# vislearn/esac

Hardware: NVIDIA H100
Metric: pose hypotheses scored/sec (640x480, 256 hyp x E experts) (higher is better)
Workload: dtype f32 (scoring) / f64 (P3P, refinement)

## Files before the change

esac_b200/csrc/esac_p3p_fast.cuh:

```cuda
#pragma once
#include "esac_geom.cuh"

namespace esacb200 {

struct Pack1 {
    float a;
    static constexpr int W = 1;
};
struct Mask1 {
    bool a;
};
struct Pack2 {
    float2 v;
    static constexpr int W = 2;
};
struct Mask2 {
    bool a, b;
};
template <typename P> struct MaskOf;
template <> struct MaskOf<Pack1> { typedef Mask1 type; };
template <> struct MaskOf<Pack2> { typedef Mask2 type; };

ESAC_HD Pack1 bc1(float x) { Pack1 r; r.a = x; return r; }
ESAC_HD Pack2 bc2(float x) { Pack2 r; r.v = make_float2(x, x); return r; }
template <typename P> ESAC_HD P bc(float x);
template <> ESAC_HD Pack1 bc<Pack1>(float x) { return bc1(x); }
template <> ESAC_HD Pack2 bc<Pack2>(float x) { return bc2(x); }

ESAC_HD Pack1 operator+(Pack1 x, Pack1 y) { return bc1(x.a + y.a); }
ESAC_HD Pack1 operator-(Pack1 x, Pack1 y) { return bc1(x.a - y.a); }
ESAC_HD Pack1 operator*(Pack1 x, Pack1 y) { return bc1(x.a * y.a); }
ESAC_HD Pack1 operator-(Pack1 x) { return bc1(-x.a); }
ESAC_HD Pack1 fma_(Pack1 x, Pack1 y, Pack1 z) { return bc1(fmaf(x.a, y.a, z.a)); }
#ifdef __CUDA_ARCH__
ESAC_HD Pack2 operator+(Pack2 x, Pack2 y) { Pack2 r; r.v = fadd2(x.v, y.v); return r; }
ESAC_HD Pack2 operator*(Pack2 x, Pack2 y) { Pack2 r; r.v = fmul2(x.v, y.v); return r; }
ESAC_HD Pack2 fma_(Pack2 x, Pack2 y, Pack2 z) { Pack2 r; r.v = ffma2(x.v, y.v, z.v); return r; }
ESAC_HD Pack2 operator-(Pack2 x, Pack2 y) { Pack2 r; r.v = ffma2(make_float2(-1.f, -1.f), y.v, x.v); return r; }
#else
ESAC_HD Pack2 operator+(Pack2 x, Pack2 y) { Pack2 r; r.v = make_float2(x.v.x + y.v.x, x.v.y + y.v.y); return r; }
ESAC_HD Pack2 operator*(Pack2 x, Pack2 y) { Pack2 r; r.v = make_float2(x.v.x * y.v.x, x.v.y * y.v.y); return r; }
ESAC_HD Pack2 fma_(Pack2 x, Pack2 y, Pack2 z) { Pack2 r; r.v = make_float2(fmaf(x.v.x, y.v.x, z.v.x), fmaf(x.v.y, y.v.y, z.v.y)); return r; }
ESAC_HD Pack2 operator-(Pack2 x, Pack2 y) { Pack2 r; r.v = make_float2(x.v.x - y.v.x, x.v.y - y.v.y); return r; }
#endif
ESAC_HD Pack2 operator-(Pack2 x) { Pack2 r; r.v = make_float2(-x.v.x, -x.v.y); return r; }

#define ESAC_PACK_UNARY(name, expr)                                                     \
    ESAC_HD Pack1 name(Pack1 p) { float x = p.a; return bc1(expr); }                    \
    ESAC_HD Pack2 name(Pack2 p) { Pack2 r; float x = p.v.x; r.v.x = (expr); x = p.v.y; r.v.y = (expr); return r; }
ESAC_PACK_UNARY(abs_, fabsf(x))
ESAC_PACK_UNARY(rcp_, Num<float>::div_(1.f, x))
ESAC_PACK_UNARY(sqrt_, Num<float>::sqrt_(x))
ESAC_PACK_UNARY(rsqrt_, rsqrtf(x))
ESAC_PACK_UNARY(cbrt_, cbrtf(x))
#undef ESAC_PACK_UNARY
ESAC_HD Pack1 max_(Pack1 x, Pack1 y) { return bc1(fmaxf(x.a, y.a)); }
ESAC_HD Pack1 min_(Pack1 x, Pack1 y) { return bc1(fminf(x.a, y.a)); }
ESAC_HD Pack2 max_(Pack2 x, Pack2 y) { Pack2 r; r.v = make_float2(fmaxf(x.v.x, y.v.x), fmaxf(x.v.y, y.v.y)); return r; }
ESAC_HD Pack2 min_(Pack2 x, Pack2 y) { Pack2 r; r.v = make_float2(fminf(x.v.x, y.v.x), fminf(x.v.y, y.v.y)); return r; }

#define ESAC_PACK_CMP(name, op)                                                       \
    ESAC_HD Mask1 name(Pack1 x, Pack1 y) { Mask1 m; m.a = x.a op y.a; return m; }     \
    ESAC_HD Mask2 name(Pack2 x, Pack2 y) { Mask2 m; m.a = x.v.x op y.v.x; m.b = x.v.y op y.v.y; return m; }
ESAC_PACK_CMP(lt_, <)
ESAC_PACK_CMP(le_, <=)
ESAC_PACK_CMP(gt_, >)
ESAC_PACK_CMP(ge_, >=)
#undef ESAC_PACK_CMP
ESAC_HD Mask1 operator&(Mask1 x, Mask1 y) { Mask1 m; m.a = x.a && y.a; return m; }
ESAC_HD Mask1 operator|(Mask1 x, Mask1 y) { Mask1 m; m.a = x.a || y.a; return m; }
ESAC_HD Mask1 operator!(Mask1 x) { Mask1 m; m.a = !x.a; return m; }
ESAC_HD Mask2 operator&(Mask2 x, Mask2 y) { Mask2 m; m.a = x.a && y.a; m.b = x.b && y.b; return m; }
ESAC_HD Mask2 operator|(Mask2 x, Mask2 y) { Mask2 m; m.a = x.a || y.a; m.b = x.b || y.b; return m; }
ESAC_HD Mask2 operator!(Mask2 x) { Mask2 m; m.a = !x.a; m.b = !x.b; return m; }
ESAC_HD Mask1 mask1(bool v) { Mask1 m; m.a = v; return m; }
ESAC_HD Mask2 mask2(bool v) { Mask2 m; m.a = v; m.b = v; return m; }
template <typename M> ESAC_HD M splat(bool v);
template <> ESAC_HD Mask1 splat<Mask1>(bool v) { return mask1(v); }
template <> ESAC_HD Mask2 splat<Mask2>(bool v) { return mask2(v); }
ESAC_HD bool all_(Mask1 m) { return m.a; }
ESAC_HD bool all_(Mask2 m) { return m.a && m.b; }
ESAC_HD Pack1 sel(Mask1 m, Pack1 x, Pack1 y) { return bc1(m.a ? x.a : y.a); }
ESAC_HD Pack2 sel(Mask2 m, Pack2 x, Pack2 y) { Pack2 r; r.v = make_float2(m.a ? x.v.x : y.v.x, m.b ? x.v.y : y.v.y); return r; }
ESAC_HD Mask1 nan_(Pack1 x) { return mask1(!(x.a == x.a)); }
ESAC_HD Mask2 nan_(Pack2 x) { Mask2 m; m.a = !(x.v.x == x.v.x); m.b = !(x.v.y == x.v.y); return m; }

template <typename P, typename M>
ESAC_HD void argmax3(P a0, P a1, P a2, M& is0, M& is1) {
    is0 = ge_(a0, a1) & ge_(a0, a2);
    is1 = !is0 & ge_(a1, a2);
}
template <typename P, typename M>
ESAC_HD P sel3(M is0, M is1, P v0, P v1, P v2) { return sel(is0, v0, sel(is1, v1, v2)); }

template <typename P, typename M>
ESAC_HD void fast_line_conic(P l0, P l1, P l2, P d00, P d01, P d02, P d11, P d12, P d22, P o[2][3], M& ok, M& unc) {
    using N = Num<float>;
    const P zero = bc<P>(0.f), one = bc<P>(1.f), two = bc<P>(2.f);
    const P a0 = abs_(l0), a1 = abs_(l1), a2 = abs_(l2);
    M k0, k1;
    argmax3(a0, a1, a2, k0, k1);
    const P li = sel3(k0, k1, l1, l2, l0), lj = sel3(k0, k1, l2, l0, l1), lk = sel3(k0, k1, l0, l1, l2);
    const M lk_ok = gt_(abs_(lk), zero);
    const P Dii = sel3(k0, k1, d11, d22, d00), Djj = sel3(k0, k1, d22, d00, d11), Dkk = sel3(k0, k1, d00, d11, d22);
    const P Dij = sel3(k0, k1, d12, d02, d01), Dik = sel3(k0, k1, d01, d12, d02), Djk = sel3(k0, k1, d02, d01, d12);
    const P ilk = rcp_(lk);
    const P r = li * ilk, s = lj * ilk;
    const P A = Dii - two * r * Dik + r * r * Dkk;
    const P B = Dij - s * Dik - r * Djk + r * s * Dkk;
    const P C = Djj - two * s * Djk + s * s * Dkk;
    P disc = B * B - A * C;
    const P mag = B * B + abs_(A * C);
    unc = unc | !lk_ok | (lk_ok & lt_(abs_(disc), bc<P>(N::kUncertain) * mag));
    const M real = !lt_(disc, -(bc<P>(N::kDiscTol) * mag));
    disc = max_(disc, zero);
    const P sq = sqrt_(disc);
    const P q = -(B + sel(ge_(B, zero), sq, -sq));
    const M useA = ge_(abs_(A), abs_(C));
    const P den = sel(useA, A, C), oth = sel(useA, C, A);
    const M den_ok = gt_(abs_(den), zero);
    unc = unc | (lk_ok & real & !den_ok);
    const P r0 = q * rcp_(den);
    const M q_nz = !(ge_(q, zero) & le_(q, zero));
    const P r1 = sel(q_nz, oth * rcp_(q), r0);
    ok = lk_ok & real & den_ok;
#pragma unroll
    for (int t = 0; t < 2; ++t) {
        const P rt = t == 0 ? r0 : r1;
        const P al = sel(useA, rt, one), be = sel(useA, one, rt);
        const P vi = al, vj = be, vk = -(r * al) - s * be;
        o[t][0] = sel3(k0, k1, vk, vj, vi);
        o[t][1] = sel3(k0, k1, vi, vk, vj);
        o[t][2] = sel3(k0, k1, vj, vi, vk);
    }
}

constexpr float kPrefilterMargin = 2.f;
constexpr float kPrefilterNeedle = 0.02f;

template <typename P>
ESAC_HD typename MaskOf<P>::type p3p_may_pass_pack(const P obj[4][3], const P img[4][2], float f, float ppx, float ppy, float tau,
                                                   float margin = kPrefilterMargin, float needle = kPrefilterNeedle) {
    typedef typename MaskOf<P>::type M;
    using N = Num<float>;
    const P zero = bc<P>(0.f), one = bc<P>(1.f), two = bc<P>(2.f);
    M decided = splat<M>(false), verdict = splat<M>(false);
#define ESAC_LATCH(cond, value)                         \
    {                                                   \
        const M c_ = (cond) & !decided;                 \
        verdict = (verdict & !c_) | (c_ & (value));     \
        decided = decided | c_;                         \
    }
    const M yes = splat<M>(true), no = splat<M>(false);
    P y[3][3], x1[3], x2[3], x3[3];
    const P ifx = bc<P>(N::div_(1.f, f)), vppx = bc<P>(ppx), vppy = bc<P>(ppy);
#pragma unroll
    for (int i = 0; i < 3; ++i) {
        const P bx = (img[i][0] - vppx) * ifx, by = (img[i][1] - vppy) * ifx;
        const P n = rsqrt_(fma_(bx, bx, fma_(by, by, one)));
        y[i][0] = bx * n; y[i][1] = by * n; y[i][2] = n;
    }
#pragma unroll
    for (int c = 0; c < 3; ++c) { x1[c] = obj[1][c] - obj[0][c]; x2[c] = obj[2][c] - obj[0][c]; x3[c] = obj[3][c] - obj[0][c]; }
    const P a12 = x1[0] * x1[0] + x1[1] * x1[1] + x1[2] * x1[2];
    const P a13 = x2[0] * x2[0] + x2[1] * x2[1] + x2[2] * x2[2];
    const P e0 = x1[0] - x2[0], e1 = x1[1] - x2[1], e2 = x1[2] - x2[2];
    const P a23 = e0 * e0 + e1 * e1 + e2 * e2;
    const P amax = max_(a12, max_(a13, a23)), amin = min_(a12, min_(a13, a23));
    ESAC_LATCH(nan_(amax), yes)
    ESAC_LATCH(!gt_(amax, zero), no)
    ESAC_LATCH(!lt_(amax, bc<P>(1e30f)), yes)
    const P c12 = y[0][0] * y[1][0] + y[0][1] * y[1][1] + y[0][2] * y[1][2];
    const P c13 = y[0][0] * y[2][0] + y[0][1] * y[2][1] + y[0][2] * y[2][2];
    const P c23 = y[1][0] * y[2][0] + y[1][1] * y[2][1] + y[1][2] * y[2][2];
    const P cm = max_(abs_(c12), max_(abs_(c13), abs_(c23)));
    ESAC_LATCH(lt_(amin, bc<P>(needle) * amax) | gt_(cm, bc<P>(0.9999f)), yes)
    const P iam = rcp_(amax);
    const P s12 = a12 * iam, s13 = a13 * iam, s23 = a23 * iam;
    const P p00 = s23, p01 = -(s23 * c12), p11 = s23 - s12, p12 = s12 * c23, p22 = -s12;
    const P q00 = s23, q02 = -(s23 * c13), q11 = -s13, q12 = s13 * c23, q22 = s23 - s13;
    const P P00 = p11 * p22 - p12 * p12, P01 = -(p01 * p22), P02 = p01 * p12;
    const P P11 = p00 * p22, P12 = -(p00 * p12), P22 = p00 * p11 - p01 * p01;
    const P Q00 = q11 * q22 - q12 * q12, Q01 = q02 * q12, Q02 = -(q02 * q11);
    const P Q11 = q00 * q22 - q02 * q02, Q12 = -(q00 * q12), Q22 = q00 * q11;
    const P k0 = p00 * P00 + p01 * P01;
    const P k3 = q00 * Q00 + q02 * Q02;
    const P k1 = P00 * q00 + P11 * q11 + P22 * q22 + two * (P02 * q02 + P12 * q12);
    const P k2 = Q00 * p00 + Q11 * p11 + Q22 * p22 + two * (Q01 * p01 + Q12 * p12);
    const P ksc = abs_(k3) + abs_(k2) + abs_(k1) + abs_(k0);
    ESAC_LATCH(!gt_(abs_(k3), bc<P>(1e-4f) * ksc), yes)
    const P ik3 = rcp_(k3);
    const P a = k2 * ik3, b = k1 * ik3, c = k0 * ik3;
    const P three = bc<P>(3.f);
    const P Qq = (a * a - three * b) * bc<P>(1.f / 9.f);
    const P Rr = (two * a * a * a - bc<P>(9.f) * a * b + bc<P>(27.f) * c) * bc<P>(1.f / 54.f);
    const P m3 = max_(sqrt_(abs_(Qq)), cbrt_(abs_(Rr)));
    P t = sel(gt_(Rr, zero), bc<P>(-2.002f), bc<P>(2.002f)) * m3;
#pragma unroll
    for (int it = 0; it < 10; ++it) {
        const P fv = (t * t - three * Qq) * t + two * Rr, dv = three * (t * t - Qq);
        t = t - sel(gt_(abs_(dv), zero), fv * rcp_(dv), zero);
    }
    P g = t - a * bc<P>(1.f / 3.f);
    {
        const P fv = ((g + a) * g + b) * g + c, dv = (three * g + two * a) * g + b;
        g = g - sel(gt_(abs_(dv), zero), fv * rcp_(dv), zero);
    }
    ESAC_LATCH(nan_(g), yes)
    const M small = le_(abs_(g), one);
    const P w1 = sel(small, one, rcp_(g)), w2 = sel(small, g, one);
    const P d00 = w1 * p00 + w2 * q00, d01 = w1 * p01, d02 = w2 * q02;
    const P d11 = w1 * p11 + w2 * q11, d12 = w1 * p12 + w2 * q12, d22 = w1 * p22 + w2 * q22;
    const P o00 = sel(small, q00, p00), o01 = sel(small, zero, p01), o02 = sel(small, q02, zero);
    const P o11 = sel(small, q11, p11), o12 = sel(small, q12, p12), o22 = sel(small, q22, p22);
    const P B00 = d11 * d22 - d12 * d12, B01 = d02 * d12 - d01 * d22, B02 = d01 * d12 - d02 * d11;
    const P B11 = d00 * d22 - d02 * d02, B12 = d01 * d02 - d00 * d12, B22 = d00 * d11 - d01 * d01;
    M ib0, ib1;
    argmax3(abs_(B00), abs_(B11), abs_(B22), ib0, ib1);
    const P bii = sel3(ib0, ib1, B00, B11, B22);
    const P nD = abs_(d00) + abs_(d11) + abs_(d22) + two * (abs_(d01) + abs_(d02) + abs_(d12));
    ESAC_LATCH(gt_(abs_(d00 * B00 + d01 * B01 + d02 * B02), bc<P>(1e-4f) * nD * nD * nD), yes)
    ESAC_LATCH(lt_(abs_(bii), bc<P>(N::kUncertain) * nD * nD), yes)
    ESAC_LATCH(!lt_(bii, zero), no)
    const P isq = rsqrt_(-bii);
    const P pv0 = sel3(ib0, ib1, B00, B01, B02) * isq, pv1 = sel3(ib0, ib1, B01, B11, B12) * isq, pv2 = sel3(ib0, ib1, B02, B12, B22) * isq;
    const P Cm[3][3] = {{d00, d01 - pv2, d02 + pv1}, {d01 + pv2, d11, d12 - pv0}, {d02 - pv1, d12 + pv0, d22}};
    P best = bc<P>(-1.f);
    P L0 = zero, L1 = zero, L2 = zero, M0 = zero, M1 = zero, M2 = zero;
#pragma unroll
    for (int r = 0; r < 3; ++r)
#pragma unroll
        for (int cc = 0; cc < 3; ++cc) {
            const P v = abs_(Cm[r][cc]);
            const M up = gt_(v, best);
            best = sel(up, v, best);
            L0 = sel(up, Cm[r][0], L0); L1 = sel(up, Cm[r][1], L1); L2 = sel(up, Cm[r][2], L2);
            M0 = sel(up, Cm[0][cc], M0); M1 = sel(up, Cm[1][cc], M1); M2 = sel(up, Cm[2][cc], M2);
        }
    ESAC_LATCH(!gt_(best, zero), yes)
    P dir[4][3];
    M unc = no, okL, okM;
    fast_line_conic(L0, L1, L2, o00, o01, o02, o11, o12, o22, &dir[0], okL, unc);
    fast_line_conic(M0, M1, M2, o00, o01, o02, o11, o12, o22, &dir[2], okM, unc);
    ESAC_LATCH(unc, yes)
    ESAC_LATCH(!okL & !okM, no)
    P nrm[3];
    nrm[0] = x1[1] * x2[2] - x1[2] * x2[1];
    nrm[1] = x1[2] * x2[0] - x1[0] * x2[2];
    nrm[2] = x1[0] * x2[1] - x1[1] * x2[0];
    const P g12 = x1[0] * x2[0] + x1[1] * x2[1] + x1[2] * x2[2];
    const P nn = nrm[0] * nrm[0] + nrm[1] * nrm[1] + nrm[2] * nrm[2];
    const P det = a12 * a13 - g12 * g12;
    ESAC_LATCH(!gt_(det, bc<P>(1e-6f) * a12 * a13) | !gt_(nn, zero), yes)
    const P v1 = x3[0] * x1[0] + x3[1] * x1[1] + x3[2] * x1[2], v2 = x3[0] * x2[0] + x3[1] * x2[1] + x3[2] * x2[2];
    const P idet = rcp_(det);
    const P al = (v1 * a13 - v2 * g12) * idet, be = (v2 * a12 - v1 * g12) * idet;
    const P ga = (x3[0] * nrm[0] + x3[1] * nrm[1] + x3[2] * nrm[2]) * rcp_(nn);
    const float lim = margin * tau;
    const P lim2 = bc<P>(lim * lim);
    const P sa = sqrt_(amax);
    const P vf = bc<P>(f);
    M pass = no;
#pragma unroll
    for (int s = 0; s < 4; ++s) {
        const M live = s < 2 ? okL : okM;
        P l0 = dir[s][0], l1 = dir[s][1], l2 = dir[s][2];
        const P q12 = l0 * l0 + l1 * l1 - two * c12 * l0 * l1;
        const P q13 = l0 * l0 + l2 * l2 - two * c13 * l0 * l2;
        const P q23 = l1 * l1 + l2 * l2 - two * c23 * l1 * l2;
        const M m12 = ge_(q12, q13) & ge_(q12, q23), m13 = !m12 & ge_(q13, q23);
        const P sc2 = sel3(m12, m13, s12, s13, s23) * rcp_(sel3(m12, m13, q12, q13, q23));
        const M scale_ok = gt_(sc2, zero) & lt_(sc2, bc<P>(1e30f));
        P sc = sqrt_(sc2);
        const P mx = max_(abs_(l0), max_(abs_(l1), abs_(l2)));
        const P ku = bc<P>(N::kUncertain) * mx;
        const M near0 = lt_(abs_(l0), ku) | lt_(abs_(l1), ku) | lt_(abs_(l2), ku);
        const M pos3 = gt_(l0, zero) & gt_(l1, zero) & gt_(l2, zero), neg3 = lt_(l0, zero) & lt_(l1, zero) & lt_(l2, zero);
        sc = sel(neg3, -sc, sc);
        const M signs_ok = pos3 | neg3;
        pass = pass | (live & scale_ok & near0);
        const M use = live & scale_ok & signs_ok;
        l0 = l0 * sc; l1 = l1 * sc; l2 = l2 * sc;
        const P res = abs_(l0 * l0 + l1 * l1 - two * c12 * l0 * l1 - s12) + abs_(l0 * l0 + l2 * l2 - two * c13 * l0 * l2 - s13) +
                      abs_(l1 * l1 + l2 * l2 - two * c23 * l1 * l2 - s23);
        pass = pass | (use & !lt_(res, bc<P>(1e-4f) * (l0 * l0 + l1 * l1 + l2 * l2 + one)));
        P P0[3], u1[3], u2[3], m[3];
#pragma unroll
        for (int cc = 0; cc < 3; ++cc) {
            P0[cc] = l0 * sa * y[0][cc];
            u1[cc] = l1 * sa * y[1][cc] - P0[cc];
            u2[cc] = l2 * sa * y[2][cc] - P0[cc];
        }
        m[0] = u1[1] * u2[2] - u1[2] * u2[1];
        m[1] = u1[2] * u2[0] - u1[0] * u2[2];
        m[2] = u1[0] * u2[1] - u1[1] * u2[0];
        const P xc = P0[0] + al * u1[0] + be * u2[0] + ga * m[0];
        const P yc = P0[1] + al * u1[1] + be * u2[1] + ga * m[1];
        const P zc = P0[2] + al * u1[2] + be * u2[2] + ga * m[2];
        const P iz = rcp_(zc);
        const P du = vppx + vf * xc * iz - img[3][0], dv = vppy + vf * yc * iz - img[3][1];
        const P e = du * du + dv * dv;
        pass = pass | (use & !gt_(e, lim2));
    }
    ESAC_LATCH(yes, pass)
#undef ESAC_LATCH
    return verdict;
}

ESAC_HD bool p3p_may_pass_fast(const float obj[4][3], const float img[4][2], float f, float ppx, float ppy, float tau,
                               float margin = kPrefilterMargin, float needle = kPrefilterNeedle) {
    Pack1 o[4][3], im[4][2];
#pragma unroll
    for (int i = 0; i < 4; ++i) {
#pragma unroll
        for (int c = 0; c < 3; ++c) o[i][c] = bc1(obj[i][c]);
        im[i][0] = bc1(img[i][0]); im[i][1] = bc1(img[i][1]);
    }
    return p3p_may_pass_pack<Pack1>(o, im, f, ppx, ppy, tau, margin, needle).a;
}

ESAC_HD void p3p_may_pass_fast2(const float obj0[4][3], const float img0[4][2], const float obj1[4][3], const float img1[4][2], float f,
                                float ppx, float ppy, float tau, bool& pass0, bool& pass1, float margin = kPrefilterMargin,
                                float needle = kPrefilterNeedle) {
    Pack2 o[4][3], im[4][2];
#pragma unroll
    for (int i = 0; i < 4; ++i) {
#pragma unroll
        for (int c = 0; c < 3; ++c) o[i][c].v = make_float2(obj0[i][c], obj1[i][c]);
        im[i][0].v = make_float2(img0[i][0], img1[i][0]);
        im[i][1].v = make_float2(img0[i][1], img1[i][1]);
    }
    const Mask2 m = p3p_may_pass_pack<Pack2>(o, im, f, ppx, ppy, tau, margin, needle);
    pass0 = m.a; pass1 = m.b;
}

}
```

esac_b200/csrc/hyp.cu:

```cuda
#include "esac_internal.h"
#include "esac_p3p_fast.cuh"
#include "esac_rng.cuh"

#include <type_traits>

namespace esacb200 {

constexpr int kTryThreads = 128;
constexpr int kNoTry = 0x7fffffff;
constexpr unsigned long long kNoKey = ~0ull;
constexpr unsigned kNoSlot = 0xffffffffu;
constexpr int kTraceWaves = 32;

struct SampleArgs {
    const float4* coords4;
    const int* assign32;
    Problem P;
    uint64_t seed;
    int limit;
    const int* injected;
    int inj_T;
    int use_prefilter;
    int hyp_offset;
    int hyp_stride;
    int h_first, h_step, Mg;
    const int* perm;
    const int* offsets;
    int e_lo, e_hi;
    int span0;
    float window;
    float tail_boost;
    SampleState st;
    unsigned long long* trace;
    int trace_slot;
};
struct SampleArgsDev : SampleArgs {
    DevParams dev;
};
template <bool DEV>
using SampleArgsT = std::conditional_t<DEV, SampleArgsDev, SampleArgs>;

template <bool DEV>
__device__ __forceinline__ uint64_t sample_seed(const SampleArgsT<DEV>& a) {
    if constexpr (DEV) {
        const uint64_t base = __ldg(a.dev.seed), calls = __ldg(a.dev.seed + 1) + (uint64_t)a.dev.index;
        if (calls == 0 || a.dev.fixed_seed) return base;
        return mix64(base + kGold * calls);
    } else {
        return a.seed;
    }
}

__device__ __forceinline__ unsigned long long gtime() {
    unsigned long long t;
    asm volatile("mov.u64 %0, %globaltimer;" : "=l"(t));
    return t;
}
struct TraceScope {
    unsigned long long* p;
    __device__ TraceScope(const unsigned long long* base, int slot) : p(nullptr) {
        if (base && threadIdx.x == 0) { p = const_cast<unsigned long long*>(base) + 2 * slot; atomicMin(p, gtime()); }
    }
    __device__ ~TraceScope() { if (p) atomicMax(p + 1, gtime()); }
};

__device__ __forceinline__ int lane_size(const SampleArgs& a) {
    return a.perm ? a.offsets[a.e_hi] - a.offsets[a.e_lo] : a.Mg;
}
__device__ __forceinline__ int lane_hyp(const SampleArgs& a, int k) {
    return a.perm ? a.perm[a.offsets[a.e_lo] + k] : a.h_first + k * a.h_step;
}

template <bool DEV>
__device__ __forceinline__ void load_try(const SampleArgsT<DEV>& a, int h, int t, int cx[4], int cy[4], float obj[4][3], float img[4][2]) {
    const Problem& P = a.P;
    if (a.injected) {
        const int* c = a.injected + ((size_t)h * a.inj_T + t) * 8;
        for (int j = 0; j < 4; ++j) { cx[j] = c[2 * j]; cy[j] = c[2 * j + 1]; }
    } else {
        draw_minimal_set(sample_seed<DEV>(a), (uint32_t)(h * a.hyp_stride + a.hyp_offset), (uint32_t)t, P.W, P.H, cx, cy);
    }
    const float4* pl = a.coords4 + (size_t)a.assign32[h] * P.N;
    for (int j = 0; j < 4; ++j) {
        const int p = cy[j] * P.W + cx[j];
        const float4 v = __ldg(pl + p);
        obj[j][0] = v.x; obj[j][1] = v.y; obj[j][2] = v.z;
        img[j][0] = (float)(cx[j] * P.sub + P.sub / 2 - dev_shift_x<DEV>(P, a));
        img[j][1] = (float)(cy[j] * P.sub + P.sub / 2 - dev_shift_y<DEV>(P, a));
    }
}

template <bool DEV>
__device__ __noinline__ bool exact_try(const SampleArgsT<DEV>& a, int h, int t, Pose& pose, int cx[4], int cy[4], bool& solved,
                                       bool verdict_only = false) {
    float obj[4][3], img[4][2];
    load_try<DEV>(a, h, t, cx, cy, obj, img);
    if constexpr (DEV) {
        const double f = (double)dev_f<DEV>(a.P, a), ppx = (double)dev_ppx<DEV>(a.P, a), ppy = (double)dev_ppy<DEV>(a.P, a);
        solved = p3p_pose(obj, img, f, ppx, ppy, pose, verdict_only ? 1.25 * (double)a.P.tau + 1. : 0.);
        return solved && minimal_set_gate(obj, img, pose, f, ppx, ppy, a.P.tau);
    } else {
        const double f = (double)a.P.f, ppx = (double)a.P.ppx, ppy = (double)a.P.ppy;
        solved = p3p_pose(obj, img, f, ppx, ppy, pose, verdict_only ? 1.25 * (double)a.P.tau + 1. : 0.);
        return solved && minimal_set_gate(obj, img, pose, f, ppx, ppy, a.P.tau);
    }
}

__global__ void interleave_kernel(const float* __restrict__ coords, float4* __restrict__ out, int E, int N) {
    const size_t total = (size_t)E * N;
    for (size_t i = (size_t)blockIdx.x * blockDim.x + threadIdx.x; i < total; i += (size_t)gridDim.x * blockDim.x) {
        const size_t e = i / N, p = i - e * N;
        const float* pl = coords + e * 3 * (size_t)N;
        out[i] = make_float4(pl[p], pl[N + p], pl[2 * (size_t)N + p], 0.f);
    }
}

__global__ void sample_init_kernel(const __grid_constant__ SampleArgs a) {
    const SampleState& st = a.st;
    const int k = blockIdx.x * blockDim.x + threadIdx.x;
    const int n = lane_size(a);
    if (k < n) {
        const int h = lane_hyp(a, k);
        st.best[h] = kNoKey; st.base[h] = 0; st.ovf[h] = kNoTry; st.list[k] = h;
    }
    if (k == 0) {
        st.counters[0] = n; st.counters[1] = 0; st.counters[2] = 0; st.counters[3] = a.span0; st.counters[4] = 0;
        st.counters[5] = 0; st.counters[6] = 0; st.counters[7] = 0;
    }
}

constexpr int kPackTries = 2 * kTryThreads;
struct PreItem {
    int h, ta, tb;
    bool valid0, valid1;
    unsigned cell[8];
};
__device__ __forceinline__ void cp_async16(void* smem, const void* gmem) {
    asm volatile("cp.async.ca.shared.global [%0], [%1], 16;" ::"r"((unsigned)__cvta_generic_to_shared(smem)), "l"(gmem) : "memory");
}
template <bool DEV>
__device__ __forceinline__ void prefilter_issue(const SampleArgsT<DEV>& a, long long item, int cph, int span, float4 (*dst)[kTryThreads], PreItem& it) {
    const int u = (int)(item / cph), c = (int)(item - (long long)u * cph);
    it.h = a.st.list[u];
    const int t0 = a.st.base[it.h];
    const int off0 = c * kPackTries + threadIdx.x, off1 = off0 + kTryThreads;
    it.valid0 = off0 < span && t0 + off0 < a.limit;
    it.valid1 = off1 < span && t0 + off1 < a.limit;
    it.ta = it.valid0 ? t0 + off0 : t0;
    it.tb = it.valid1 ? t0 + off1 : t0;
    if (!(it.valid0 || it.valid1)) return;
    const Problem& P = a.P;
    const float4* pl = a.coords4 + (size_t)a.assign32[it.h] * P.N;
#pragma unroll
    for (int k = 0; k < 2; ++k) {
        const int t = k == 0 ? it.ta : it.tb;
        int cx[4], cy[4];
        if (a.injected) {
            const int* cc = a.injected + ((size_t)it.h * a.inj_T + t) * 8;
            for (int j = 0; j < 4; ++j) { cx[j] = cc[2 * j]; cy[j] = cc[2 * j + 1]; }
        } else {
            draw_minimal_set(sample_seed<DEV>(a), (uint32_t)(it.h * a.hyp_stride + a.hyp_offset), (uint32_t)t, P.W, P.H, cx, cy);
        }
#pragma unroll
        for (int j = 0; j < 4; ++j) {
            it.cell[k * 4 + j] = ((unsigned)cy[j] << 16) | (unsigned)cx[j];
            cp_async16(&dst[k * 4 + j][threadIdx.x], pl + (cy[j] * P.W + cx[j]));
        }
    }
}

template <bool DEV>
__global__ void __launch_bounds__(kTryThreads, 4) prefilter_kernel(const __grid_constant__ SampleArgsT<DEV> a) {
    TraceScope trace(a.trace, a.trace_slot);
    __shared__ float4 s_obj[2][8][kTryThreads];
    const int n_unres = a.st.counters[0];
    const int span = a.st.counters[3];
    const int cph = (span + kPackTries - 1) / kPackTries;
    const long long n_items = (long long)n_unres * cph;
    const int lane = threadIdx.x & 31, tid = threadIdx.x;
    const Problem& P = a.P;
    PreItem cur, nxt;
    long long item = blockIdx.x;
    if (item < n_items) prefilter_issue<DEV>(a, item, cph, span, s_obj[0], cur);
    asm volatile("cp.async.commit_group;" ::: "memory");
    int buf = 0;
    for (; item < n_items; item += gridDim.x) {
        const long long ni = item + gridDim.x;
        if (ni < n_items) prefilter_issue<DEV>(a, ni, cph, span, s_obj[buf ^ 1], nxt);
        asm volatile("cp.async.commit_group;" ::: "memory");
        asm volatile("cp.async.wait_group 1;" ::: "memory");
        bool pass0 = false, pass1 = false;
        if (cur.valid0 || cur.valid1) {
            float obj0[4][3], img0[4][2], obj1[4][3], img1[4][2];
#pragma unroll
            for (int j = 0; j < 4; ++j) {
                const float4 v0 = s_obj[buf][j][tid], v1 = s_obj[buf][4 + j][tid];
                obj0[j][0] = v0.x; obj0[j][1] = v0.y; obj0[j][2] = v0.z;
                obj1[j][0] = v1.x; obj1[j][1] = v1.y; obj1[j][2] = v1.z;
                const unsigned c0 = cur.cell[j], c1 = cur.cell[4 + j];
                img0[j][0] = (float)((int)(c0 & 0xffffu) * P.sub + P.sub / 2 - dev_shift_x<DEV>(P, a));
                img0[j][1] = (float)((int)(c0 >> 16) * P.sub + P.sub / 2 - dev_shift_y<DEV>(P, a));
                img1[j][0] = (float)((int)(c1 & 0xffffu) * P.sub + P.sub / 2 - dev_shift_x<DEV>(P, a));
                img1[j][1] = (float)((int)(c1 >> 16) * P.sub + P.sub / 2 - dev_shift_y<DEV>(P, a));
            }
            if (a.use_prefilter)
                p3p_may_pass_fast2(obj0, img0, obj1, img1, dev_f<DEV>(P, a), dev_ppx<DEV>(P, a), dev_ppy<DEV>(P, a), P.tau,
                                   pass0, pass1);
            else pass0 = pass1 = true;
            pass0 = pass0 && cur.valid0;
            pass1 = pass1 && cur.valid1;
        }
        const unsigned m0 = __ballot_sync(0xffffffffu, pass0), m1 = __ballot_sync(0xffffffffu, pass1);
        if (m0 | m1) {
            const int n0 = __popc(m0);
            int basei = 0;
            if (lane == 0) basei = atomicAdd(&a.st.counters[1], n0 + __popc(m1));
            basei = __shfl_sync(0xffffffffu, basei, 0);
            const unsigned lt = (1u << lane) - 1u;
            if (pass0) {
                const int idx = basei + __popc(m0 & lt);
                if (idx < a.st.cap) a.st.surv[idx] = make_int2(cur.h, cur.ta);
                else atomicMin(&a.st.ovf[cur.h], cur.ta);
            }
            if (pass1) {
                const int idx = basei + n0 + __popc(m1 & lt);
                if (idx < a.st.cap) a.st.surv[idx] = make_int2(cur.h, cur.tb);
                else atomicMin(&a.st.ovf[cur.h], cur.tb);
            }
        }
        cur = nxt;
        buf ^= 1;
    }
    asm volatile("cp.async.wait_group 0;" ::: "memory");
}

__device__ void advance_wave(const SampleState& st, int limit, float window, float tail_boost);

template <bool DEV>
__global__ void __launch_bounds__(128) exact_kernel(const __grid_constant__ SampleArgsT<DEV> a) {
    TraceScope trace(a.trace, a.trace_slot);
    const int n = min(a.st.counters[1], a.st.cap);
    for (int i = blockIdx.x * blockDim.x + threadIdx.x; i < n; i += gridDim.x * blockDim.x) {
        const int2 ht = a.st.surv[i];
        if (ht.y >= a.st.ovf[ht.x]) continue;
        Pose pose;
        int cx[4], cy[4];
        bool solved;
        if (exact_try<DEV>(a, ht.x, ht.y, pose, cx, cy, solved, true)) {
            unsigned slot = (unsigned)atomicAdd(&a.st.counters[2], 1);
            if (slot < (unsigned)a.st.cap_acc) {
                Accepted& ac = a.st.stage[slot];
                ac.pose = pose;
                for (int j = 0; j < 4; ++j) { ac.cells[2 * j] = cx[j]; ac.cells[2 * j + 1] = cy[j]; }
            } else {
                slot = kNoSlot;
            }
            atomicMin(&a.st.best[ht.x], ((unsigned long long)(unsigned)ht.y << 32) | slot);
        }
    }
    __shared__ int s_last;
    __threadfence();
    __syncthreads();
    if (threadIdx.x == 0) s_last = atomicAdd(&a.st.counters[4], 1) == (int)gridDim.x - 1;
    __syncthreads();
    if (s_last) {
        __threadfence();
        advance_wave(a.st, a.limit, a.window, a.tail_boost);
    }
}

__device__ void advance_wave(const SampleState& st, int limit, float window, float tail_boost) {
    __shared__ int s_fill;
    const int span = st.counters[3];
    if (threadIdx.x == 0) s_fill = 0;
    __syncthreads();
    const int n_unres = st.counters[0];
    int* next = st.list + st.M;
    for (int u = threadIdx.x; u < n_unres; u += blockDim.x) {
        const int h = st.list[u];
        const int ovf = st.ovf[h];
        const int end = min(st.base[h] + span, ovf);
        const unsigned long long best = __ldcg(&st.best[h]);
        const bool resolved = (long long)(best >> 32) < (long long)end;
        if (!resolved) {
            if (best != kNoKey) st.best[h] = kNoKey;
            st.base[h] = end;
            st.ovf[h] = kNoTry;
            if (end < limit) next[atomicAdd(&s_fill, 1)] = h;
        }
    }
    __syncthreads();
    const int nn = s_fill;
    for (int u = threadIdx.x; u < nn; u += blockDim.x) st.list[u] = next[u];
    __syncthreads();
    if (threadIdx.x == 0) {
        const int n_surv = min(st.counters[1], st.cap);
        const double tried = (double)n_unres * (double)span;
        const double hits = n_unres - nn > 0 ? (double)(n_unres - nn) : 0.5;
        const double boost = nn <= 8 ? tail_boost * 2. : (nn <= 64 ? tail_boost : 1.);
        double next_span = (double)window * boost * tried / hits;
        next_span = next_span < 256. ? 256. : (next_span > 65536. ? 65536. : next_span);
        st.counters[3] = ((int)next_span + kPackTries - 1) / kPackTries * kPackTries;
        st.counters[0] = nn;
        st.counters[1] = 0;
        st.counters[4] = 0;
        if (n_unres > 0) {
            st.counters[5] += n_unres * span;
            st.counters[6] += n_surv;
            st.counters[7] += 1;
        }
    }
}

template <bool DEV>
__global__ void __launch_bounds__(kTryThreads) tail_kernel(const __grid_constant__ SampleArgsT<DEV> a) {
    const int n_unres = a.st.counters[0];
    __shared__ int s_list[kTryThreads * 8];
    __shared__ int s_n, s_best;
    for (int u = blockIdx.x; u < n_unres; u += gridDim.x) {
        const int h = a.st.list[u];
        int base = a.st.base[h];
        __syncthreads();
        if (threadIdx.x == 0) s_best = kNoTry;
        while (base < a.limit) {
            if (threadIdx.x == 0) s_n = 0;
            __syncthreads();
            const int span = min(a.limit - base, kTryThreads * 8);
            for (int t = base + threadIdx.x; t < base + span; t += kTryThreads) {
                int cx[4], cy[4];
                float obj[4][3], img[4][2];
                load_try<DEV>(a, h, t, cx, cy, obj, img);
                if (!a.use_prefilter ||
                    p3p_may_pass_fast(obj, img, dev_f<DEV>(a.P, a), dev_ppx<DEV>(a.P, a), dev_ppy<DEV>(a.P, a), a.P.tau))
                    s_list[atomicAdd(&s_n, 1)] = t;
            }
            __syncthreads();
            const int n = s_n;
            for (int i = threadIdx.x; i < n; i += kTryThreads) {
                Pose pose;
                int cx[4], cy[4];
                bool solved;
                if (exact_try<DEV>(a, h, s_list[i], pose, cx, cy, solved, true)) atomicMin(&s_best, s_list[i]);
            }
            __syncthreads();
            if (s_best != kNoTry) break;
            base += span;
        }
        if (threadIdx.x == 0 && s_best != kNoTry) a.st.best[h] = ((unsigned long long)(unsigned)s_best << 32) | kNoSlot;
    }
}


template <bool DEV>
__global__ void __launch_bounds__(64) emit_kernel(const __grid_constant__ SampleArgsT<DEV> a, Pose* poses, int* cells, int* tries) {
    const int k = blockIdx.x * blockDim.x + threadIdx.x;
    if (k >= lane_size(a)) return;
    const int h = lane_hyp(a, k);
    const unsigned long long key = a.st.best[h];
    const int t = key != kNoKey ? (int)(key >> 32) : a.limit - 1;
    const unsigned slot = (unsigned)(key & 0xffffffffu);
    Pose pose;
    int cx[4], cy[4];
    if (key != kNoKey && slot != kNoSlot) {
        const Accepted& ac = a.st.stage[slot];
        pose = ac.pose;
        for (int j = 0; j < 4; ++j) { cx[j] = ac.cells[2 * j]; cy[j] = ac.cells[2 * j + 1]; }
    } else {
        bool solved;
        exact_try<DEV>(a, h, t, pose, cx, cy, solved);
        if (!solved) { for (int c = 0; c < 3; ++c) { pose.r[c] = 0; pose.t[c] = 0; } }
    }
    poses[h] = pose;
    for (int j = 0; j < 4; ++j) { cells[h * 8 + 2 * j] = cx[j]; cells[h * 8 + 2 * j + 1] = cy[j]; }
    tries[h] = t + 1;
}

int launch_sample(const float* coords, float4* coords4, const int* assign32, const Problem& P, uint64_t seed, int max_tries,
                  const int* injected, int inj_T, const SampleState* st, int n_lanes, int sm_count, int use_prefilter,
                  int hyp_offset, int hyp_stride, Pose* poses, int* cells, int* tries, const cudaStream_t* lanes,
                  cudaEvent_t ev_fork, const cudaEvent_t* ev_join, int split_e, const int* perm, const int* offsets,
                  const cudaEvent_t* ev_half, int span0, float window, int n_waves,
                  unsigned long long* trace, float tail_boost, const DevParams* dev) {
    int launches = 0;
    cudaStream_t stream = lanes[0];
    if (!split_e) { interleave_kernel<<<sm_count * 8, 256, 0, stream>>>(coords, coords4, P.E, P.N); ++launches; }
    SampleArgsDev args[4];
    int bound[4];
    for (int g = 0; g < n_lanes; ++g) {
        SampleArgsDev& a = args[g];
        a.coords4 = coords4; a.assign32 = assign32; a.P = P; a.seed = seed;
        a.limit = injected ? (max_tries < inj_T ? max_tries : inj_T) : max_tries;
        a.injected = injected; a.inj_T = inj_T; a.st = st[g]; a.use_prefilter = use_prefilter; a.hyp_offset = hyp_offset; a.hyp_stride = hyp_stride > 0 ? hyp_stride : 1;
        a.h_first = g; a.h_step = n_lanes; a.Mg = (P.M - g + n_lanes - 1) / n_lanes;
        a.perm = nullptr; a.offsets = nullptr; a.e_lo = a.e_hi = 0;
        a.span0 = span0; a.window = window; a.trace = trace; a.trace_slot = 0; a.tail_boost = tail_boost;
        a.dev = dev ? *dev : DevParams{};
        bound[g] = a.Mg;
        if (split_e) {
            a.perm = perm; a.offsets = offsets;
            a.e_lo = g == 0 ? 0 : split_e;
            a.e_hi = g == 0 ? split_e : P.E;
            bound[g] = P.M;
        }
    }
    if (n_lanes > 1) {
        cudaEventRecord(ev_fork, stream);
        for (int g = 1; g < n_lanes; ++g) cudaStreamWaitEvent(lanes[g], ev_fork, 0);
    }
    for (int g = 0; g < n_lanes; ++g) {
        cudaStream_t sg = lanes[g];
        SampleArgsDev& a = args[g];
        const SampleArgs& ae = a;
        if (split_e) {
            cudaStreamWaitEvent(sg, ev_half[g], 0);
            const int ne = a.e_hi - a.e_lo;
            interleave_kernel<<<sm_count * 8, 256, 0, sg>>>(coords + (size_t)a.e_lo * 3 * P.N, coords4 + (size_t)a.e_lo * P.N, ne, P.N);
            ++launches;
        }
        if (bound[g] <= 0) continue;
        sample_init_kernel<<<(bound[g] + 255) / 256, 256, 0, sg>>>(ae); ++launches;
        const int grid = sm_count * 4;
        for (int r = 0; r < n_waves; ++r) {
            a.trace = r < kTraceWaves ? trace : nullptr;
            a.trace_slot = (g * kTraceWaves + r) * 2;
            if (dev) prefilter_kernel<true><<<grid, kTryThreads, 0, sg>>>(a);
            else prefilter_kernel<false><<<grid, kTryThreads, 0, sg>>>(ae);
            ++launches;
            a.trace_slot = (g * kTraceWaves + r) * 2 + 1;
            if (dev) exact_kernel<true><<<sm_count * 4, 128, 0, sg>>>(a);
            else exact_kernel<false><<<sm_count * 4, 128, 0, sg>>>(ae);
            ++launches;
        }
        const int tail_grid = bound[g] < sm_count * 4 ? bound[g] : sm_count * 4;
        if (dev) {
            tail_kernel<true><<<tail_grid, kTryThreads, 0, sg>>>(a);
            emit_kernel<true><<<(bound[g] + 63) / 64, 64, 0, sg>>>(a, poses, cells, tries);
        } else {
            tail_kernel<false><<<tail_grid, kTryThreads, 0, sg>>>(ae);
            emit_kernel<false><<<(bound[g] + 63) / 64, 64, 0, sg>>>(ae, poses, cells, tries);
        }
        launches += 2;
    }
    for (int g = 1; g < n_lanes; ++g) {
        cudaEventRecord(ev_join[g], lanes[g]);
        cudaStreamWaitEvent(stream, ev_join[g], 0);
    }
    return launches;
}

__global__ void trace_init_kernel(unsigned long long* trace, int slots) {
    const int i = blockIdx.x * blockDim.x + threadIdx.x;
    if (i < slots) { trace[2 * i] = ~0ull; trace[2 * i + 1] = 0ull; }
}
void launch_trace_init(unsigned long long* trace, int slots, cudaStream_t st) { trace_init_kernel<<<(slots + 255) / 256, 256, 0, st>>>(trace, slots); }

}
```

Measured before the change: 902,100.

## Drop packed two-hypothesis prefilter for scalar one-try-per-thread with higher occupancy

The prefilter kernel no longer evaluates two P3P minimal sets per thread using packed float2 arithmetic. Each thread now handles one try, which halves the per-thread shared-memory staging and register state. Launch bounds and grid size are raised from 4 to 6 blocks per SM to use the freed resources. On H100 the packed FFMA2 helpers may not map to native paired instructions, so the packing mostly added register pressure; the trade-off is more items and more loop overhead per try.

```diff
diff --git a/esac_b200/csrc/esac_p3p_fast.cuh b/esac_b200/csrc/esac_p3p_fast.cuh
--- a/esac_b200/csrc/esac_p3p_fast.cuh
+++ b/esac_b200/csrc/esac_p3p_fast.cuh
@@ -10,44 +10,21 @@
 struct Mask1 {
     bool a;
 };
-struct Pack2 {
-    float2 v;
-    static constexpr int W = 2;
-};
-struct Mask2 {
-    bool a, b;
-};
 template <typename P> struct MaskOf;
 template <> struct MaskOf<Pack1> { typedef Mask1 type; };
-template <> struct MaskOf<Pack2> { typedef Mask2 type; };
 
 ESAC_HD Pack1 bc1(float x) { Pack1 r; r.a = x; return r; }
-ESAC_HD Pack2 bc2(float x) { Pack2 r; r.v = make_float2(x, x); return r; }
 template <typename P> ESAC_HD P bc(float x);
 template <> ESAC_HD Pack1 bc<Pack1>(float x) { return bc1(x); }
-template <> ESAC_HD Pack2 bc<Pack2>(float x) { return bc2(x); }
 
 ESAC_HD Pack1 operator+(Pack1 x, Pack1 y) { return bc1(x.a + y.a); }
 ESAC_HD Pack1 operator-(Pack1 x, Pack1 y) { return bc1(x.a - y.a); }
 ESAC_HD Pack1 operator*(Pack1 x, Pack1 y) { return bc1(x.a * y.a); }
 ESAC_HD Pack1 operator-(Pack1 x) { return bc1(-x.a); }
 ESAC_HD Pack1 fma_(Pack1 x, Pack1 y, Pack1 z) { return bc1(fmaf(x.a, y.a, z.a)); }
-#ifdef __CUDA_ARCH__
-ESAC_HD Pack2 operator+(Pack2 x, Pack2 y) { Pack2 r; r.v = fadd2(x.v, y.v); return r; }
-ESAC_HD Pack2 operator*(Pack2 x, Pack2 y) { Pack2 r; r.v = fmul2(x.v, y.v); return r; }
-ESAC_HD Pack2 fma_(Pack2 x, Pack2 y, Pack2 z) { Pack2 r; r.v = ffma2(x.v, y.v, z.v); return r; }
-ESAC_HD Pack2 operator-(Pack2 x, Pack2 y) { Pack2 r; r.v = ffma2(make_float2(-1.f, -1.f), y.v, x.v); return r; }
-#else
-ESAC_HD Pack2 operator+(Pack2 x, Pack2 y) { Pack2 r; r.v = make_float2(x.v.x + y.v.x, x.v.y + y.v.y); return r; }
-ESAC_HD Pack2 operator*(Pack2 x, Pack2 y) { Pack2 r; r.v = make_float2(x.v.x * y.v.x, x.v.y * y.v.y); return r; }
-ESAC_HD Pack2 fma_(Pack2 x, Pack2 y, Pack2 z) { Pack2 r; r.v = make_float2(fmaf(x.v.x, y.v.x, z.v.x), fmaf(x.v.y, y.v.y, z.v.y)); return r; }
-ESAC_HD Pack2 operator-(Pack2 x, Pack2 y) { Pack2 r; r.v = make_float2(x.v.x - y.v.x, x.v.y - y.v.y); return r; }
-#endif
-ESAC_HD Pack2 operator-(Pack2 x) { Pack2 r; r.v = make_float2(-x.v.x, -x.v.y); return r; }
-
-#define ESAC_PACK_UNARY(name, expr)                                                     \
-    ESAC_HD Pack1 name(Pack1 p) { float x = p.a; return bc1(expr); }                    \
-    ESAC_HD Pack2 name(Pack2 p) { Pack2 r; float x = p.v.x; r.v.x = (expr); x = p.v.y; r.v.y = (expr); return r; }
+
+#define ESAC_PACK_UNARY(name, expr) \
+    ESAC_HD Pack1 name(Pack1 p) { float x = p.a; return bc1(expr); }
 ESAC_PACK_UNARY(abs_, fabsf(x))
 ESAC_PACK_UNARY(rcp_, Num<float>::div_(1.f, x))
 ESAC_PACK_UNARY(sqrt_, Num<float>::sqrt_(x))
@@ -56,12 +33,9 @@
 #undef ESAC_PACK_UNARY
 ESAC_HD Pack1 max_(Pack1 x, Pack1 y) { return bc1(fmaxf(x.a, y.a)); }
 ESAC_HD Pack1 min_(Pack1 x, Pack1 y) { return bc1(fminf(x.a, y.a)); }
-ESAC_HD Pack2 max_(Pack2 x, Pack2 y) { Pack2 r; r.v = make_float2(fmaxf(x.v.x, y.v.x), fmaxf(x.v.y, y.v.y)); return r; }
-ESAC_HD Pack2 min_(Pack2 x, Pack2 y) { Pack2 r; r.v = make_float2(fminf(x.v.x, y.v.x), fminf(x.v.y, y.v.y)); return r; }
-
-#define ESAC_PACK_CMP(name, op)                                                       \
-    ESAC_HD Mask1 name(Pack1 x, Pack1 y) { Mask1 m; m.a = x.a op y.a; return m; }     \
-    ESAC_HD Mask2 name(Pack2 x, Pack2 y) { Mask2 m; m.a = x.v.x op y.v.x; m.b = x.v.y op y.v.y; return m; }
+
+#define ESAC_PACK_CMP(name, op) \
+    ESAC_HD Mask1 name(Pack1 x, Pack1 y) { Mask1 m; m.a = x.a op y.a; return m; }
 ESAC_PACK_CMP(lt_, <)
 ESAC_PACK_CMP(le_, <=)
 ESAC_PACK_CMP(gt_, >)
@@ -70,20 +44,12 @@
 ESAC_HD Mask1 operator&(Mask1 x, Mask1 y) { Mask1 m; m.a = x.a && y.a; return m; }
 ESAC_HD Mask1 operator|(Mask1 x, Mask1 y) { Mask1 m; m.a = x.a || y.a; return m; }
 ESAC_HD Mask1 operator!(Mask1 x) { Mask1 m; m.a = !x.a; return m; }
-ESAC_HD Mask2 operator&(Mask2 x, Mask2 y) { Mask2 m; m.a = x.a && y.a; m.b = x.b && y.b; return m; }
-ESAC_HD Mask2 operator|(Mask2 x, Mask2 y) { Mask2 m; m.a = x.a || y.a; m.b = x.b || y.b; return m; }
-ESAC_HD Mask2 operator!(Mask2 x) { Mask2 m; m.a = !x.a; m.b = !x.b; return m; }
 ESAC_HD Mask1 mask1(bool v) { Mask1 m; m.a = v; return m; }
-ESAC_HD Mask2 mask2(bool v) { Mask2 m; m.a = v; m.b = v; return m; }
 template <typename M> ESAC_HD M splat(bool v);
 template <> ESAC_HD Mask1 splat<Mask1>(bool v) { return mask1(v); }
-template <> ESAC_HD Mask2 splat<Mask2>(bool v) { return mask2(v); }
 ESAC_HD bool all_(Mask1 m) { return m.a; }
-ESAC_HD bool all_(Mask2 m) { return m.a && m.b; }
 ESAC_HD Pack1 sel(Mask1 m, Pack1 x, Pack1 y) { return bc1(m.a ? x.a : y.a); }
-ESAC_HD Pack2 sel(Mask2 m, Pack2 x, Pack2 y) { Pack2 r; r.v = make_float2(m.a ? x.v.x : y.v.x, m.b ? x.v.y : y.v.y); return r; }
 ESAC_HD Mask1 nan_(Pack1 x) { return mask1(!(x.a == x.a)); }
-ESAC_HD Mask2 nan_(Pack2 x) { Mask2 m; m.a = !(x.v.x == x.v.x); m.b = !(x.v.y == x.v.y); return m; }
 
 template <typename P, typename M>
 ESAC_HD void argmax3(P a0, P a1, P a2, M& is0, M& is1) {
@@ -319,19 +285,4 @@
     return p3p_may_pass_pack<Pack1>(o, im, f, ppx, ppy, tau, margin, needle).a;
 }
 
-ESAC_HD void p3p_may_pass_fast2(const float obj0[4][3], const float img0[4][2], const float obj1[4][3], const float img1[4][2], float f,
-                                float ppx, float ppy, float tau, bool& pass0, bool& pass1, float margin = kPrefilterMargin,
-                                float needle = kPrefilterNeedle) {
-    Pack2 o[4][3], im[4][2];
-#pragma unroll
-    for (int i = 0; i < 4; ++i) {
-#pragma unroll
-        for (int c = 0; c < 3; ++c) o[i][c].v = make_float2(obj0[i][c], obj1[i][c]);
-        im[i][0].v = make_float2(img0[i][0], img1[i][0]);
-        im[i][1].v = make_float2(img0[i][1], img1[i][1]);
-    }
-    const Mask2 m = p3p_may_pass_pack<Pack2>(o, im, f, ppx, ppy, tau, margin, needle);
-    pass0 = m.a; pass1 = m.b;
-}
-
-}
+}
diff --git a/esac_b200/csrc/hyp.cu b/esac_b200/csrc/hyp.cu
--- a/esac_b200/csrc/hyp.cu
+++ b/esac_b200/csrc/hyp.cu
@@ -129,11 +129,11 @@
     }
 }
 
-constexpr int kPackTries = 2 * kTryThreads;
+constexpr int kSpanQuantum = 256;
 struct PreItem {
-    int h, ta, tb;
-    bool valid0, valid1;
-    unsigned cell[8];
+    int h, t;
+    bool valid;
+    unsigned cell[4];
 };
 __device__ __forceinline__ void cp_async16(void* smem, const void* gmem) {
     asm volatile("cp.async.ca.shared.global [%0], [%1], 16;" ::"r"((unsigned)__cvta_generic_to_shared(smem)), "l"(gmem) : "memory");
@@ -143,39 +143,33 @@
     const int u = (int)(item / cph), c = (int)(item - (long long)u * cph);
     it.h = a.st.list[u];
     const int t0 = a.st.base[it.h];
-    const int off0 = c * kPackTries + threadIdx.x, off1 = off0 + kTryThreads;
-    it.valid0 = off0 < span && t0 + off0 < a.limit;
-    it.valid1 = off1 < span && t0 + off1 < a.limit;
-    it.ta = it.valid0 ? t0 + off0 : t0;
-    it.tb = it.valid1 ? t0 + off1 : t0;
-    if (!(it.valid0 || it.valid1)) return;
+    const int off = c * kTryThreads + threadIdx.x;
+    it.t = t0 + off;
+    it.valid = off < span && it.t < a.limit;
+    if (!it.valid) return;
     const Problem& P = a.P;
     const float4* pl = a.coords4 + (size_t)a.assign32[it.h] * P.N;
+    int cx[4], cy[4];
+    if (a.injected) {
+        const int* cc = a.injected + ((size_t)it.h * a.inj_T + it.t) * 8;
+        for (int j = 0; j < 4; ++j) { cx[j] = cc[2 * j]; cy[j] = cc[2 * j + 1]; }
+    } else {
+        draw_minimal_set(sample_seed<DEV>(a), (uint32_t)(it.h * a.hyp_stride + a.hyp_offset), (uint32_t)it.t, P.W, P.H, cx, cy);
+    }
 #pragma unroll
-    for (int k = 0; k < 2; ++k) {
-        const int t = k == 0 ? it.ta : it.tb;
-        int cx[4], cy[4];
-        if (a.injected) {
-            const int* cc = a.injected + ((size_t)it.h * a.inj_T + t) * 8;
-            for (int j = 0; j < 4; ++j) { cx[j] = cc[2 * j]; cy[j] = cc[2 * j + 1]; }
-        } else {
-            draw_minimal_set(sample_seed<DEV>(a), (uint32_t)(it.h * a.hyp_stride + a.hyp_offset), (uint32_t)t, P.W, P.H, cx, cy);
-        }
-#pragma unroll
-        for (int j = 0; j < 4; ++j) {
-            it.cell[k * 4 + j] = ((unsigned)cy[j] << 16) | (unsigned)cx[j];
-            cp_async16(&dst[k * 4 + j][threadIdx.x], pl + (cy[j] * P.W + cx[j]));
-        }
-    }
-}
-
-template <bool DEV>
-__global__ void __launch_bounds__(kTryThreads, 4) prefilter_kernel(const __grid_constant__ SampleArgsT<DEV> a) {
+    for (int j = 0; j < 4; ++j) {
+        it.cell[j] = ((unsigned)cy[j] << 16) | (unsigned)cx[j];
+        cp_async16(&dst[j][threadIdx.x], pl + (cy[j] * P.W + cx[j]));
+    }
+}
+
+template <bool DEV>
+__global__ void __launch_bounds__(kTryThreads, 6) prefilter_kernel(const __grid_constant__ SampleArgsT<DEV> a) {
     TraceScope trace(a.trace, a.trace_slot);
-    __shared__ float4 s_obj[2][8][kTryThreads];
+    __shared__ float4 s_obj[2][4][kTryThreads];
     const int n_unres = a.st.counters[0];
     const int span = a.st.counters[3];
-    const int cph = (span + kPackTries - 1) / kPackTries;
+    const int cph = (span + kTryThreads - 1) / kTryThreads;
     const long long n_items = (long long)n_unres * cph;
     const int lane = threadIdx.x & 31, tid = threadIdx.x;
     const Problem& P = a.P;
@@ -189,43 +183,28 @@
         if (ni < n_items) prefilter_issue<DEV>(a, ni, cph, span, s_obj[buf ^ 1], nxt);
         asm volatile("cp.async.commit_group;" ::: "memory");
         asm volatile("cp.async.wait_group 1;" ::: "memory");
-        bool pass0 = false, pass1 = false;
-        if (cur.valid0 || cur.valid1) {
-            float obj0[4][3], img0[4][2], obj1[4][3], img1[4][2];
+        bool pass = false;
+        if (cur.valid) {
+            float obj[4][3], img[4][2];
 #pragma unroll
             for (int j = 0; j < 4; ++j) {
-                const float4 v0 = s_obj[buf][j][tid], v1 = s_obj[buf][4 + j][tid];
-                obj0[j][0] = v0.x; obj0[j][1] = v0.y; obj0[j][2] = v0.z;
-                obj1[j][0] = v1.x; obj1[j][1] = v1.y; obj1[j][2] = v1.z;
-                const unsigned c0 = cur.cell[j], c1 = cur.cell[4 + j];
-                img0[j][0] = (float)((int)(c0 & 0xffffu) * P.sub + P.sub / 2 - dev_shift_x<DEV>(P, a));
-                img0[j][1] = (float)((int)(c0 >> 16) * P.sub + P.sub / 2 - dev_shift_y<DEV>(P, a));
-                img1[j][0] = (float)((int)(c1 & 0xffffu) * P.sub + P.sub / 2 - dev_shift_x<DEV>(P, a));
-                img1[j][1] = (float)((int)(c1 >> 16) * P.sub + P.sub / 2 - dev_shift_y<DEV>(P, a));
+                const float4 v = s_obj[buf][j][tid];
+                obj[j][0] = v.x; obj[j][1] = v.y; obj[j][2] = v.z;
+                const unsigned c = cur.cell[j];
+                img[j][0] = (float)((int)(c & 0xffffu) * P.sub + P.sub / 2 - dev_shift_x<DEV>(P, a));
+                img[j][1] = (float)((int)(c >> 16) * P.sub + P.sub / 2 - dev_shift_y<DEV>(P, a));
             }
-            if (a.use_prefilter)
-                p3p_may_pass_fast2(obj0, img0, obj1, img1, dev_f<DEV>(P, a), dev_ppx<DEV>(P, a), dev_ppy<DEV>(P, a), P.tau,
-                                   pass0, pass1);
-            else pass0 = pass1 = true;
-            pass0 = pass0 && cur.valid0;
-            pass1 = pass1 && cur.valid1;
-        }
-        const unsigned m0 = __ballot_sync(0xffffffffu, pass0), m1 = __ballot_sync(0xffffffffu, pass1);
-        if (m0 | m1) {
-            const int n0 = __popc(m0);
+            pass = !a.use_prefilter || p3p_may_pass_fast(obj, img, dev_f<DEV>(P, a), dev_ppx<DEV>(P, a), dev_ppy<DEV>(P, a), P.tau);
+        }
+        const unsigned m = __ballot_sync(0xffffffffu, pass);
+        if (m) {
             int basei = 0;
-            if (lane == 0) basei = atomicAdd(&a.st.counters[1], n0 + __popc(m1));
+            if (lane == 0) basei = atomicAdd(&a.st.counters[1], __popc(m));
             basei = __shfl_sync(0xffffffffu, basei, 0);
-            const unsigned lt = (1u << lane) - 1u;
-            if (pass0) {
-                const int idx = basei + __popc(m0 & lt);
-                if (idx < a.st.cap) a.st.surv[idx] = make_int2(cur.h, cur.ta);
-                else atomicMin(&a.st.ovf[cur.h], cur.ta);
-            }
-            if (pass1) {
-                const int idx = basei + n0 + __popc(m1 & lt);
-                if (idx < a.st.cap) a.st.surv[idx] = make_int2(cur.h, cur.tb);
-                else atomicMin(&a.st.ovf[cur.h], cur.tb);
+            if (pass) {
+                const int idx = basei + __popc(m & ((1u << lane) - 1u));
+                if (idx < a.st.cap) a.st.surv[idx] = make_int2(cur.h, cur.t);
+                else atomicMin(&a.st.ovf[cur.h], cur.t);
             }
         }
         cur = nxt;
@@ -300,7 +279,7 @@
         const double boost = nn <= 8 ? tail_boost * 2. : (nn <= 64 ? tail_boost : 1.);
         double next_span = (double)window * boost * tried / hits;
         next_span = next_span < 256. ? 256. : (next_span > 65536. ? 65536. : next_span);
-        st.counters[3] = ((int)next_span + kPackTries - 1) / kPackTries * kPackTries;
+        st.counters[3] = ((int)next_span + kSpanQuantum - 1) / kSpanQuantum * kSpanQuantum;
         st.counters[0] = nn;
         st.counters[1] = 0;
         st.counters[4] = 0;
@@ -419,7 +398,7 @@
         }
         if (bound[g] <= 0) continue;
         sample_init_kernel<<<(bound[g] + 255) / 256, 256, 0, sg>>>(ae); ++launches;
-        const int grid = sm_count * 4;
+        const int grid = sm_count * 6;
         for (int r = 0; r < n_waves; ++r) {
             a.trace = r < kTraceWaves ? trace : nullptr;
             a.trace_slot = (g * kTraceWaves + r) * 2;
```

New measurement: 961,400, median of 6. 1.07x the previous value.
